# diffqc/dqc

Hardware: AMD Instinct MI355X
Metric: SCF iterations/sec (Fock build + XC grid) per GPU, cc-pVDZ 20-atom (higher is better)
Workload: dtype f64

## Files before the change

### dqc_amd/batch.py

```python
from typing import Callable, List, Sequence

import torch
import torch.distributed as dist


def molecule_cost(nao: int, ngrid: int) -> float:
    return float(nao) ** 4 + 12.0 * float(ngrid) * float(nao) ** 2


def molecule_bytes(nao: int, ngrid: int, ncomp: int = 4) -> int:
    nb = (nao + 7) // 8
    npair = nb * (nb + 1) // 2
    ld = (nao + 15) // 16 * 16 + 16
    return npair * (npair + 1) // 2 * 4096 * 8 + 8 * ncomp * ngrid * ld + 8 * 16 * ngrid + 64 * ld * ld


def reserve_device_memory(nbytes: int, device) -> float:
    import time
    dev = torch.device(device)
    free, _ = torch.cuda.mem_get_info(dev)
    cached = torch.cuda.memory_reserved(dev) - torch.cuda.memory_allocated(dev)
    nbytes = int(min(nbytes, free - (2 << 30)))
    if nbytes <= cached:
        return 0.0
    torch.cuda.synchronize(dev)
    t0 = time.perf_counter()
    block = torch.empty(nbytes, dtype=torch.uint8, device=dev)
    del block
    return time.perf_counter() - t0
# ... 170 lines not shown
```

### dqc_amd/csrc/common.hpp

```cpp
#pragma once
#include <hip/hip_runtime.h>
#include <cmath>
#include <cstdint>
#include <cstdio>
#include <cstring>
#include <mutex>
#include <string>
#include <vector>

#include "../../include/dqc_amd.h"

#define DQC_LMAX 4
#define DQC_TILE_B 8
#define DQC_TILE_SZ 4096

namespace dqc {

__host__ __device__ inline int tile_dim(bool diag) { return diag ? 36 : 64; }
__host__ __device__ inline int tile_pidx(bool diag, int a, int b) {
    if (!diag) return a * 8 + b;
    const int hi = a > b ? a : b, lo = a > b ? b : a;
    return hi * (hi + 1) / 2 + lo;
}
__host__ __device__ inline long long tile_row_off(long long I, long long J) {
// ... 129 lines not shown
        void *p = nullptr;
        if (dmalloc(&p, n * sizeof(T) + 8)) return DQC_ENOMEM;
        *dst = (T *)p;
        return 0;
    }
    void release() {
        for (void *p : ptrs) (void)(async ? hipFreeAsync(p, ast) : hipFree(p));
        ptrs.clear();
        for (Staging *s : stg) staging_release(s, ast);
        stg.clear();
    }
    ~DevPool() { release(); }
};

int upload_shells(DevShells &d, const Basis &b, DevPool &pool, hipStream_t st);

inline int ncart(int l) { return (l + 1) * (l + 2) / 2; }

struct SideStreams {
    static constexpr int MAX = 4;
    hipStream_t s[MAX] = {};
    hipEvent_t ev_fork = nullptr, ev_join[MAX] = {};
    int n = 0, next = 0;
    hipStream_t take() { return s[next++ % n]; }
    int fork(hipStream_t st) {
        if (hipEventRecord(ev_fork, st) != hipSuccess) return DQC_EHIP;
        for (int i = 0; i < n; i++)
            if (hipStreamWaitEvent(s[i], ev_fork, 0) != hipSuccess) return DQC_EHIP;
        return DQC_OK;
    }
// ... 172 lines not shown
```

### dqc_amd/csrc/grid_density.hip

```cpp
#include "grid_common.hpp"

namespace dqc {

constexpr int DEN_BM = 64;
constexpr int DEN_NT = DEN_BM * 4;
constexpr int DEN_KC = 16;
constexpr int DEN_SA = DEN_KC + 2;

#ifdef DEN_TRACE
__device__ long long g_den_trace[4 * 16384];
DQC_DEV void den_trace(int k) {
    if (threadIdx.x == 0 && blockIdx.x < 16384) {
        if (k == 0) {
            unsigned hw, xcc;
            asm volatile("s_getreg_b32 %0, hwreg(HW_REG_HW_ID)" : "=s"(hw));
            asm volatile("s_getreg_b32 %0, hwreg(HW_REG_XCC_ID)" : "=s"(xcc));
            g_den_trace[4 * blockIdx.x + 3] = (long long)(((xcc & 7u) << 8) | ((hw >> 8) & 0xffu));
        }
        g_den_trace[4 * blockIdx.x + k] = wall_clock64();
    }
}
#define DEN_TRACE_POINT(k) den_trace(k)
#else
#define DEN_TRACE_POINT(k)
// ... 571 lines not shown
    unsigned n = 0;
    while (__hip_atomic_load(flag, __ATOMIC_ACQUIRE, __HIP_MEMORY_SCOPE_WORKGROUP) < want) {
        if (__hip_atomic_load(broken, __ATOMIC_RELAXED, __HIP_MEMORY_SCOPE_WORKGROUP) != 0u) break;
        if (++n > ROLE_SPIN_CAP) {
            __hip_atomic_store(broken, 1u, __ATOMIC_RELAXED, __HIP_MEMORY_SCOPE_WORKGROUP);
            break;
        }
        __builtin_amdgcn_s_sleep(2);
    }
}

DQC_DEV void role_signal(unsigned *flag, unsigned v) {
    __hip_atomic_store(flag, v, __ATOMIC_RELEASE, __HIP_MEMORY_SCOPE_WORKGROUP);
}

template <int NRT, int NT>
__global__ __launch_bounds__(ROLE_NT, 1) void density_roles_kernel(double *__restrict__ rho, double *__restrict__ grho,
                                                                   const double *__restrict__ ao, int ngrid,
                                                                   const double *__restrict__ orbt, int lda) {
    using G = RoleGeom<NRT, NT>;
    constexpr int RP = G::RP, S = G::S, P0 = G::P0, P1 = G::P1, LD = NT * 16;
    constexpr int NPF = 4;
    static_assert(NT >= 2 && NT <= 14 && P1 >= 1, "one epilogue panel of 2..14 tiles");
    extern __shared__ __attribute__((aligned(16))) double lds[];
    double *sLT = lds, *sMB = lds + G::LT_SZ, *sAall = sMB + 4 * G::MB_W;
    unsigned *flags = reinterpret_cast<unsigned *>(sAall + 4 * G::SA_W);
    const int tid = threadIdx.x, lane = tid & 63;
    const int wave = __builtin_amdgcn_readfirstlane(tid >> 6);
    const int lr = lane & 15, lk = lane >> 4;
    const int ntiles = (ngrid + DEN_BM - 1) / DEN_BM;
    const size_t cs = (size_t)ngrid * lda;

    for (int e = tid; e < RP * LD; e += ROLE_NT) {
        const int r = e / LD, c = e - r * LD;
        sLT[r * S + c] = orbt[e];
    }
    if (tid < 16) flags[tid] = 0u;
    __syncthreads();
    const int w = wave & 3;
    unsigned *filled = flags + w, *drained = flags + 4 + w, *broken = flags + 8;
    double *mb = sMB + w * G::MB_W + lane * 2;
    unsigned seq = 0;

    if (wave < 4) {
        double *sA = sAall + w * G::SA_W;
        const int arow = lane >> 2, aseg = (lane & 3) * 4;
        double2 pa0a, pa0b, pa1a, pa1b, pa2a, pa2b, pa3a, pa3b;
        static_assert(NPF == 4, "four named prefetch sets");
#define DQC_ROLE_REQUEST(T, KC, SET)                                                                       \
    {                                                         \
        const int rmax_ = ngrid - 1 - (T) * DEN_BM;                                                        \
        const double *s_ = ao + (size_t)(T) * DEN_BM * lda + (min(w * 16 + arow, rmax_) * lda + aseg) + (KC) * DEN_KC; \
// ... 61 lines not shown
                    }
                role_wait(drained, seq, broken);
#pragma unroll
                for (int ct = 0; ct < PMAX; ct++)
                    if (ct < (h ? P1 : P0)) {
                        *reinterpret_cast<double2 *>(mb + (2 * ct) * 128) = make_double2(acc[ct][0], acc[ct][1]);
                        *reinterpret_cast<double2 *>(mb + (2 * ct + 1) * 128) = make_double2(acc[ct][2], acc[ct][3]);
                    }
                seq++;
                role_signal(filled, seq);
            }
        }
#undef DQC_ROLE_REQUEST4
#undef DQC_ROLE_STEP
#undef DQC_ROLE_REQUEST
    } else {
        for (int t = blockIdx.x; t < ntiles; t += gridDim.x) {
            const int g0 = t * DEN_BM;
            const int rmax = ngrid - 1 - g0;
            const double *aoblk = ao + (size_t)g0 * lda;
            int roff[4];
#pragma unroll
            for (int r = 0; r < 4; r++) roff[r] = min(w * 16 + lk + 4 * r, rmax) * lda + 2 * lr;
            v4d acc[NT];
#pragma unroll
            for (int h = 0; h < 2; h++) {
                role_wait(filled, seq + 1, broken);
#pragma unroll
                for (int ct = 0; ct < (h ? P1 : P0); ct++) {
                    const double2 lo = *reinterpret_cast<const double2 *>(mb + (2 * ct) * 128);
// ... 25 lines not shown
#pragma unroll
                for (int r = 0; r < 4; r++) {
                    const int row = g0 + w * 16 + lk + 4 * r;
                    if (row < ngrid) {
                        const double nan = __builtin_nan("");
                        grho[row] = bad ? nan : 2.0 * p[r][1];
                        grho[(size_t)ngrid + row] = bad ? nan : 2.0 * p[r][2];
                        grho[2 * (size_t)ngrid + row] = bad ? nan : 2.0 * p[r][3];
                    }
                }
            }
        }
    }
}

static bool density_roles_shape(int nrt, int ntile) { return nrt == 3 && ntile == 13; }

static bool density_roles_enabled() {
    const char *e = getenv("DQC_DENSITY_ROLES");
    return !(e && e[0] == '0');
}

static int launch_density_roles(int nrt, int ntile, hipStream_t st, double *rho, double *grho, const double *ao, int ngrid,
                                const double *orbt, int lda) {
    static int ncu = 0;
    if (ncu == 0) {
        int dev = 0, n = 0;
        if (hipGetDevice(&dev) != hipSuccess || hipDeviceGetAttribute(&n, hipDeviceAttributeMultiprocessorCount, dev) != hipSuccess || n <= 0) {
            set_error("density_roles: cannot read the device's CU count");
            return DQC_EINVAL;
        }
        ncu = n;
    }
    const int ntiles = (ngrid + DEN_BM - 1) / DEN_BM;
    if (nrt == 3 && ntile == 13) {
        constexpr size_t shm = RoleGeom<3, 13>::lds_bytes();
        static_assert(shm <= 160 * 1024, "one block has to fit the CU's LDS");
        auto kern = density_roles_kernel<3, 13>;
        (void)hipFuncSetAttribute((const void *)kern, hipFuncAttributeMaxDynamicSharedMemorySize, (int)shm);
        hipLaunchKernelGGL(kern, dim3(std::min(ntiles, ncu)), dim3(ROLE_NT), shm, st, rho, grho, ao, ngrid, orbt, lda);
        return 0;
    }
    set_error("density_roles: internal shape dispatch error");
    return DQC_EINVAL;
}

template <int NRT>
__global__ __launch_bounds__(256, 2) void density_lr_tau_kernel(double *__restrict__ rho, double *__restrict__ grho, double *__restrict__ tau,
                                                                const double *__restrict__ ao, int ngrid, int ld,
                                                                const double *__restrict__ orb, int lda) {
    extern __shared__ __attribute__((aligned(16))) double lds[];
    constexpr int RP = LrGeom<NRT>::RP, RPS = LrGeom<NRT>::RPS;
    constexpr int A_SZ = DEN_BM * DEN_SA, B_SZ = DEN_KC * RPS;
    constexpr int NL2 = (DEN_KC * RP / 2 + DEN_NT - 1) / DEN_NT;
    static_assert(NL2 <= 4, "L chunk wider than 4 double2 per thread");
    double *sA = lds, *sB = lds + 4 * A_SZ;
    const int tid = threadIdx.x, wave = tid >> 6, lane = tid & 63;
    const int lr = lane & 15, lk = lane >> 4;
    const int g0 = blockIdx.x * DEN_BM;
// ... 210 lines not shown
    const int lim = gga ? dqc::lr_max_nct(norb_pad / 16) : 16;
    const int nchunk = (ntile + lim - 1) / lim;
    const int nct = (ntile + nchunk - 1) / nchunk;
    dim3 grid((ngrid + DEN_BM - 1) / DEN_BM);
    int rc;
    if (gga && density_roles_shape(norb_pad / 16, ntile) && density_roles_enabled())
        rc = launch_density_roles(norb_pad / 16, ntile, st, d_rho, d_grho, d_ao, ngrid, d_orbt, lda);
    else
        rc = gga ? launch_density_lr<true>(norb_pad / 16, nct, grid, st, d_rho, d_grho, d_ao, ngrid, ld, d_orb, d_orbt, ntile, lda)
                 : launch_density_lr<false>(norb_pad / 16, nct, grid, st, d_rho, d_grho, d_ao, ngrid, ld, d_orb, d_orbt, ntile, lda);
    if (rc) return rc;
    DQC_CHECK_LAUNCH();
    return DQC_OK;
}

int dqc_grid_density_lr_roles(int nao, int norb_pad, int gga) {
    using namespace dqc;
    if (!gga || norb_pad <= 0 || dqc_padded_norb(norb_pad) != norb_pad) return 0;
    return density_roles_shape(norb_pad / 16, dqc_padded_nao(nao) / 16) && density_roles_enabled() ? 1 : 0;
}

int dqc_grid_density_lr_pol(double *d_rho, double *d_grho, const double *d_ao, int ncomp, int ngrid, int nao,
                            const double *d_orb, const double *d_orbt, int norb_pad_spin, void *stream) {
    using namespace dqc;
    hipStream_t st = (hipStream_t)stream;
    if (ngrid <= 0) return DQC_OK;
    if (!d_grho || ncomp < 4) { set_error("dqc_grid_density_lr_pol: needs the four AO components and the gradient output"); return DQC_EINVAL; }
    if (norb_pad_spin != 16 && norb_pad_spin != 32 && norb_pad_spin != 48 && norb_pad_spin != 64) {
        set_error("dqc_grid_density_lr_pol: norb_pad_spin must be 16, 32, 48 or 64");
        return DQC_EINVAL;
// ... 65 lines not shown
```

### dqc_amd/csrc/gto.hip

```cpp
#include "common.hpp"
#include <type_traits>

namespace dqc {

namespace gto_ce {
#define C2S_QUAL constexpr
#include "cart2sph.inc"
#undef C2S_QUAL
}

typedef double gto_v2d __attribute__((ext_vector_type(2)));
template <int DERIV>
__global__ __launch_bounds__(64) void eval_gto_kernel(double *__restrict__ out, const double *__restrict__ coords,
                                                       int ngrid, int nao, int ld, DevShells sh, int colrange) {
    constexpr int NC = DERIV == 0 ? 1 : (DERIV == 1 ? 4 : (DERIV == 2 ? 5 : 10));
    constexpr int GTO_CW = DERIV == 0 ? 16 : 8;
    __shared__ double tile[1][NC][64][GTO_CW + 1];
    constexpr int wave = 0;
    const int lane = threadIdx.x;
    const int g0 = blockIdx.x * 64;
    if (g0 >= ngrid) return;
    const int g = min(g0 + lane, ngrid - 1);
    const double px = coords[g * 3], py = coords[g * 3 + 1], pz = coords[g * 3 + 2];
    const size_t cstride = (size_t)ngrid * ld;

    const int cbeg = blockIdx.y * colrange, cend = min(cbeg + colrange, ld);
// ... 89 lines not shown
            if (nfill == GTO_CW) {
                flush(GTO_CW);
                col0 += GTO_CW;
                nfill = 0;
            }
        }
    };
    static_assert(DQC_LMAX == 4, "one shell body per accepted l");

    for (int is = 0; is < sh.nsh; is++) {
        const int l = sh.l[is], np = sh.nprim[is], po = sh.prim_off[is];
        const int a0 = sh.ao_off[is];
        if (a0 + 2 * l + 1 <= cbeg || a0 >= cend) continue;
        const double x = px - sh.xyz[is * 3], y = py - sh.xyz[is * 3 + 1], z = pz - sh.xyz[is * 3 + 2];
        const double r2 = x * x + y * y + z * z;
        double e0 = 0, e1 = 0, e2 = 0;
        for (int ip = 0; ip < np; ip++) {
            double a = sh.exps[po + ip];
            double e = sh.coefs[po + ip] * exp(-a * r2);
            e0 += e;
            e1 -= 2.0 * a * e;
            e2 += 4.0 * a * a * e;
        }
        switch (l) {
        case 0: shell(std::integral_constant<int, 0>{}, a0, x, y, z, e0, e1, e2); break;
        case 1: shell(std::integral_constant<int, 1>{}, a0, x, y, z, e0, e1, e2); break;
        case 2: shell(std::integral_constant<int, 2>{}, a0, x, y, z, e0, e1, e2); break;
        case 3: shell(std::integral_constant<int, 3>{}, a0, x, y, z, e0, e1, e2); break;
        default: shell(std::integral_constant<int, 4>{}, a0, x, y, z, e0, e1, e2); break;
        }
    }
    while (col0 + nfill < cend) {
        for (int c = 0; c < NC; c++) tile[wave][c][lane][nfill] = 0.0;
        nfill++;
        if (nfill == GTO_CW) {
            flush(GTO_CW);
            col0 += GTO_CW;
            nfill = 0;
// ... 25 lines not shown
        const int ncomp = deriv == 0 ? 1 : (deriv == 1 ? 4 : (deriv == 2 ? 5 : 10));
        const size_t body = (size_t)ncomp * (size_t)ngrid * ld, slack = dqc_ao_doubles(ncomp, ngrid, b.nao) - body;
        if (slack) DQC_HIP(hipMemsetAsync(d_out + body, 0, slack * sizeof(double), st));
        if (deriv == 0)
            hipLaunchKernelGGL(eval_gto_kernel<0>, grid, dim3(64), 0, st, d_out, d_coords, ngrid, b.nao, ld, ds, colrange);
        else if (deriv == 1)
            hipLaunchKernelGGL(eval_gto_kernel<1>, grid, dim3(64), 0, st, d_out, d_coords, ngrid, b.nao, ld, ds, colrange);
        else if (deriv == 2)
            hipLaunchKernelGGL(eval_gto_kernel<2>, grid, dim3(64), 0, st, d_out, d_coords, ngrid, b.nao, ld, ds, colrange);
        else
            hipLaunchKernelGGL(eval_gto_kernel<3>, grid, dim3(64), 0, st, d_out, d_coords, ngrid, b.nao, ld, ds, colrange);
        DQC_CHECK_LAUNCH();
    }
    return DQC_OK;
}
```

### dqc_amd/hamilton.py

```python
from collections import namedtuple
from typing import List, Optional

import os

import torch

from . import lib
from .basis import make_tables
from .linop import LinearOperator
from .utils.datastruct import AtomCGTOBasis, SpinParam, ValGrad
from .xc import LibXC

_COULOMB_SIDE = {}


def register_coulomb_side_stream(grid_stream, side_stream):
    key = (grid_stream.device.index, grid_stream.cuda_stream)
    if side_stream is None:
        _COULOMB_SIDE.pop(key, None)
    else:
        _COULOMB_SIDE[key] = side_stream


class _Memo:
# ... 238 lines not shown
                cached = (idx, int(idx.shape[0]))
                try:
                    grid._live_index_cache = cached
                except AttributeError:
                    pass
            if cached[1] < self.ngrid_full:
                self.live_index = cached[0]
                self.rgrid = self.rgrid[self.live_index].contiguous()
                self.dvolume = self.dvolume[self.live_index].contiguous()
        if self._pworld > 1:
            g = self.rgrid.shape[0]
            lo, hi = g * self._prank // self._pworld, g * (self._prank + 1) // self._pworld
            self.rgrid, self.dvolume = self.rgrid[lo:hi].contiguous(), self.dvolume[lo:hi].contiguous()
        deriv = {1: 0, 2: 1, 4: 2}[self.xcfamily]
        self._ao = lib.eval_gto(self._tab, self.rgrid, deriv)
        self.is_grid_set = True
        self.is_ao_set = True
        self.is_grad_ao_set = deriv >= 1
        self.is_lapl_ao_set = deriv == 2
        self._ao_lapl_pm = None

    def grid_select(self, x):
        return x if self.live_index is None else x[..., self.live_index]

    def grid_scatter(self, x):
        if self.live_index is None:
            return x
        out = torch.zeros(tuple(x.shape[:-1]) + (self.ngrid_full,), dtype=x.dtype, device=x.device)
        out[..., self.live_index] = x
        return out
# ... 342 lines not shown
        if not self.is_ao_set:
            raise RuntimeError("Please call `setup_grid(grid, xc)` first")
        gga = self.xcfamily in (2, 4)
        if gga and not self.is_grad_ao_set:
            raise RuntimeError("Please call `setup_grid(grid, gradlevel>=1)` to calculate the density gradient")
        fac = self._factor_of(dm)
        use_factor = fac is not None and (self.xcfamily != 4 or self.is_lapl_ao_set)
        self.grid_path_counts["factor" if use_factor else "dense"] += 1
        if use_factor and self.xcfamily == 4 and isinstance(self.xc, LibXC) and all(f[0].shape[1] <= 96 for f in fac):
            rho, grho, kin = lib.grid_density_lr_tau(self._ao, self._nao_ao, fac[0])
            for f in fac[1:]:
                r2, g2, k2 = lib.grid_density_lr_tau(self._ao, self._nao_ao, f)
                rho, grho, kin = rho + r2, grho + g2, kin + k2
            return ValGrad(value=rho, grad=grho, lapl=None, kin=kin)
        if use_factor:
            rho, grho = lib.grid_density_lr(self._ao, self._nao_ao, fac[0], gga)
            for f in fac[1:]:
                r2, g2 = lib.grid_density_lr(self._ao, self._nao_ao, f, gga)
                rho = rho + r2
                grho = None if grho is None else grho + g2
            if self.xcfamily != 4:
                return ValGrad(value=rho, grad=grho)
            gg = sum(lib.grid_density_lr(self._ao[d], self._nao_ao, f, False)[0] for d in (1, 2, 3) for f in fac)
            if isinstance(self.xc, LibXC):
                return ValGrad(value=rho, grad=grho, lapl=None, kin=gg * 0.5)
            if getattr(self, "_ao_lapl_pm", None) is None:
                self._ao_lapl_pm = (lib.ao_from(self._ao[0] + self._ao[4], self._nao_ao), lib.ao_from(self._ao[0] - self._ao[4], self._nao_ao))
            pl = sum(lib.grid_density_lr(self._ao_lapl_pm[0], self._nao_ao, f, False)[0] for f in fac)
            mi = sum(lib.grid_density_lr(self._ao_lapl_pm[1], self._nao_ao, f, False)[0] for f in fac)
            return ValGrad(value=rho, grad=grho, lapl=2.0 * (0.25 * (pl - mi) + gg), kin=gg * 0.5)
        dmdmt = (dm + dm.transpose(-2, -1)) * 0.5
        dao = lib.pad_matrix(self._unconvert_dm(dmdmt), self._ld)
        rho, grho = lib.grid_density(self._ao, self._nao_ao, dao, gga)
        if self.xcfamily != 4:
            return ValGrad(value=rho, grad=grho)
        if not self.is_lapl_ao_set:
            raise RuntimeError("Please call `setup_grid(grid, gradlevel>=2)` to calculate the density gradient")
        gg = sum(lib.grid_density_pair(self._ao[d], self._ao[d], self._nao_ao, dao) for d in (1, 2, 3))
        lb = lib.grid_density_pair(self._ao[0], self._ao[4], self._nao_ao, dao)
        return ValGrad(value=rho, grad=grho, lapl=(lb + gg) * 2, kin=gg * 0.5)

    def _dm2densinfo_pol(self, dm: SpinParam) -> SpinParam:
        if self.xcfamily == 2 and self.is_ao_set and self.is_grad_ao_set:
            fu, fd = self._factor_of(dm.u), self._factor_of(dm.d)
            if fu is not None and fd is not None and len(fu) == 1 and len(fd) == 1:
                out = lib.grid_density_lr_pol(self._ao, self._nao_ao, fu[0], fd[0])
                if out is not None:
                    self.grid_path_counts["factor"] += 2
                    self.grid_path_counts["factor_spin_fused"] = self.grid_path_counts.get("factor_spin_fused", 0) + 1
                    rho, grho = out
                    return SpinParam(u=ValGrad(value=rho[0], grad=grho[0]), d=ValGrad(value=rho[1], grad=grho[1]))
        return SpinParam(u=self._dm2densinfo(dm.u), d=self._dm2densinfo(dm.d))

    def _get_vxc_from_potinfo(self, potinfo: ValGrad):
        return self._sym_orth(self._vxc_ao_from_potinfo(potinfo)[:self._nao_ao, :self._nao_ao])

# ... 191 lines not shown
```

### dqc_amd/lib.py

```python
import ctypes
import os

import numpy as np
import torch

_HERE = os.path.dirname(os.path.abspath(__file__))
_LIBPATH = os.environ.get("DQC_AMD_LIB") or os.path.join(_HERE, "libdqc_amd.so")
_lib = None

XC_IDS = {"lda_x": 1, "lda_c_vwn": 7, "lda_c_pw": 12, "lda_c_pw_mod": 13, "gga_x_pbe": 101, "gga_x_pbe_r": 102, "gga_x_b88": 106,
          "gga_x_pbe_sol": 116, "gga_x_rpbe": 117, "gga_c_pbe": 130, "gga_c_lyp": 131, "gga_c_pbe_sol": 133,
          "mgga_x_scan": 263, "mgga_c_scan": 267, "mgga_x_tpss": 202, "mgga_c_tpss": 231,
          "lda_c_pz": 9, "gga_x_b86": 103, "gga_x_g96": 107, "gga_x_pw86": 108, "gga_x_pw91": 109, "gga_x_optx": 110, "gga_x_wc": 118,
          "gga_c_p86": 132}


class DqcAmdError(RuntimeError):
    pass


def libpath():
    return _LIBPATH


# ... 58 lines not shown
    lib.dqc_orth_factor_batched.argtypes = [c_dp, c_dp, c_dp, c_int, c_int, c_int, c_vp]
    lib.dqc_diis_solve.argtypes = [c_dp, c_dp, c_int, c_int, c_int, c_vp]
    lib.dqc_diis_solve_dev.argtypes = [c_dp, c_dp, c_int, c_int, c_vp, c_vp]
    lib.dqc_projector_work_doubles.argtypes = [c_int, c_int]
    lib.dqc_projector_work_doubles.restype = c_sz
    lib.dqc_projector_tc2.argtypes = [c_dp, c_dp, c_dp, c_int, ctypes.c_double, c_int, ctypes.c_double, c_dp, c_vp]
    lib.dqc_purify_tc2_persist.argtypes = [c_dp, c_dp, c_int, ctypes.c_double, c_int, ctypes.c_double, c_dp, c_vp, c_vp]
    lib.dqc_df_coulomb.argtypes = [c_dp, c_dp, c_dp, c_dp, c_int, c_int, c_dp, c_vp]
    lib.dqc_eri_tiles_to_dense.argtypes = [c_dp, c_dp, c_int, c_vp]
    lib.dqc_jk_from_tiles.argtypes = [c_dp, c_dp, c_dp, c_dp, c_int, c_dp, c_vp]
    lib.dqc_jk_multi_work_doubles.argtypes = [c_int, c_int, c_int]
    lib.dqc_jk_multi_work_doubles.restype = c_sz
    lib.dqc_jk_from_tiles_multi.argtypes = [c_dp, c_dp, c_int, c_dp, c_dp, c_int, c_dp, c_int, c_dp, c_vp]
    lib.dqc_eval_gto.argtypes = [c_int, c_dp, c_dp, c_int] + tab + [c_vp]
    lib.dqc_grid_density.argtypes = [c_dp, c_dp, c_dp, c_int, c_int, c_int, c_dp, c_vp]
    lib.dqc_xc_eval.argtypes = [c_dp, c_dp, c_dp, c_dp, c_dp, c_int, ip, dp, c_int, c_vp]
    lib.dqc_xc_eval_quad.argtypes = [c_dp, c_dp, c_dp, c_dp, c_dp, c_dp, c_dp, c_int, ip, dp, c_int, c_vp]
    lib.dqc_xc_eval_pol.argtypes = [c_dp] * 9 + [c_int, ip, dp, c_int, c_vp]
    lib.dqc_xc_eval_mgga.argtypes = [c_dp] * 7 + [c_int, ip, dp, c_int, c_vp]
    lib.dqc_xc_eval_mgga_pol.argtypes = [c_dp] * 11 + [c_int, ip, dp, c_int, c_vp]
    lib.dqc_xc_eval_mgga_pol2.argtypes = [c_dp] * 12 + [c_int, ip, dp, c_int, c_vp]
    lib.dqc_stream_create_partition.argtypes = [ctypes.POINTER(c_vp), c_int, c_int, c_int]
    lib.dqc_stream_destroy.argtypes = [c_vp]
    lib.dqc_stream_cus.argtypes = [c_vp]
    lib.dqc_set_vxc_cus.argtypes = [c_int]
    lib.dqc_fock_factor.argtypes = [c_dp, c_dp, c_dp, c_dp, c_int, c_dp, c_int, c_int, c_int, c_int, c_int, c_vp]
    lib.dqc_fock_orb2dm.argtypes = [c_dp, c_dp, c_dp, c_dp, c_dp, c_int, c_dp, c_int, c_int, c_int, c_int, c_int, c_vp]
    lib.dqc_grid_vxc_raw.argtypes = [c_dp, c_dp, c_int, c_int, c_int, c_dp, c_dp, c_dp, dp, c_vp]
    lib.dqc_fock_finish_vraw.argtypes = [c_dp, c_dp, c_dp, c_dp, c_int, ctypes.c_double, c_dp, c_dp, c_int, c_int, c_vp]
    lib.dqc_fock_prep.argtypes = [c_dp, c_dp, c_dp, c_dp, c_int, c_int, c_int, c_int, c_vp]
# ... 540 lines not shown

def eval_gto(tab, rgrid, deriv):
    ngrid = rgrid.shape[0]
    ncomp = {0: 0, 1: 4, 2: 5, 3: 10}[deriv]
    nc = max(ncomp, 1)
    lda = ao_stride(tab.nao)
    flat = torch.empty(int(load().dqc_ao_doubles(nc, int(ngrid), int(tab.nao))), dtype=torch.float64, device=rgrid.device)
    out = flat[:nc * ngrid * lda].view(nc, ngrid, lda)
    out = out[0] if ncomp == 0 else out
    with _on(rgrid.device) as st_:
        _check(load().dqc_eval_gto(deriv, _ptr(out), _ptr(rgrid.contiguous()), ngrid, *tab.args(), st_),
               "dqc_eval_gto")
    return out


def pad_matrix(m, ld):
    n = m.shape[-1]
    if n == ld:
        return m.contiguous()
    out = torch.zeros((ld, ld), dtype=m.dtype, device=m.device)
    out[:n, :n] = m
    return out


def grid_density(ao, nao, dm_pad, gga):
    ncomp = 1 if ao.dim() == 2 else ao.shape[0]
    ngrid = ao.shape[-2]
    rho = torch.empty(ngrid, dtype=torch.float64, device=ao.device)
    grho = torch.empty((3, ngrid), dtype=torch.float64, device=ao.device) if gga else None
    with _on(ao.device) as st_:
# ... 277 lines not shown
```

### include/dqc_amd.h

```cpp
#ifndef DQC_AMD_H
#define DQC_AMD_H
#include <stddef.h>
#include <stdint.h>

#ifdef __cplusplus
extern "C" {
#endif

#define DQC_OK 0
#define DQC_EINVAL (-1)
#define DQC_EHIP (-2)
#define DQC_ENOMEM (-3)

const char *dqc_last_error(void);
int dqc_version(void);
int dqc_nao(const int *bas, int nbas);
int dqc_padded_nao(int nao);
int dqc_ao_stride(int nao);
size_t dqc_ao_doubles(int ncomp, int ngrid, int nao);

int dqc_int1e(int which, double *d_out, const int *atm, int natm, const int *bas, int nbas,
              const double *env, int nenv, const double *zs, void *stream);

size_t dqc_eri_tile_count(int nao);
// ... 118 lines not shown
int dqc_orth_factor(double *d_q, const double *d_y, const double *d_g, int n, int r, void *stream);

int dqc_purify_tc2_batched(double *d_x, double *d_tmp, int ld, int nmol, double nocc, int iters, double tol,
                           double *d_state, void *stream);
int dqc_orth_factor_batched(double *d_q, const double *d_y, const double *d_g, int n, int r, int nmol, void *stream);
int dqc_diis_solve(double *d_c, const double *d_gram, int nmol, int nhist, int m, void *stream);
int dqc_diis_solve_dev(double *d_c, const double *d_gram, int nmol, int nhist, const long long *d_count, void *stream);

int dqc_grid_vxc(double *d_vmat, const double *d_ao, int ncomp, int ngrid, int nao,
                 const double *d_w, const double *d_vrho, const double *d_vgrad, void *stream);

int dqc_padded_norb(int norb);
int dqc_grid_density_lr(double *d_rho, double *d_grho, const double *d_ao, int ncomp, int ngrid, int nao,
                        const double *d_orb, const double *d_orbt, int norb_pad, void *stream);
int dqc_grid_density_lr_roles(int nao, int norb_pad, int gga);
int dqc_grid_density_lr_pol(double *d_rho, double *d_grho, const double *d_ao, int ncomp, int ngrid, int nao,
                            const double *d_orb, const double *d_orbt, int norb_pad_spin, void *stream);

int dqc_grid_xc_gradient_terms(double *d_q, double *d_perao, const double *d_ao, int ngrid, int nao, const double *d_b,
                               const double *d_c0, const double *d_c1, const double *d_c2, int ldb, const double *d_w,
                               const double *d_vrho, const double *d_u, const double *d_grho, const double *d_vtau, void *stream);

int dqc_grid_density_lr_tau(double *d_rho, double *d_grho, double *d_tau, const double *d_ao, int ncomp, int ngrid, int nao,
                            const double *d_orb, int norb_pad, void *stream);

int dqc_grid_density_pair(double *d_out, const double *d_ao_a, const double *d_ao_b, int ngrid, int nao,
                          const double *d_dm, void *stream);
int dqc_grid_vxc_pair(double *d_vmat, const double *d_ao_a, const double *d_ao_b, int ngrid, int nao,
                      const double *d_w, const double *d_v, void *stream);

// ... 40 lines not shown
```

Baseline: 796.4.

## Compute density gradient from cached radial GTO terms instead of AO gradient tables

Adds a radial table (per grid point and shell slot, the contracted exponential and its derivative) evaluated once at grid setup. A new variant of the roles density kernel rebuilds the angular derivative parts on the fly from point coordinates and compile-time cart-to-spherical coefficients, then dots them with the orbital-factor products. This avoids streaming the three AO gradient components from memory on each SCF iteration. The cost is extra arithmetic per point and extra LDS for the table, and the path only applies to one padded shape (13 tiles, l<=2, GGA).

```diff
diff --git a/dqc_amd/batch.py b/dqc_amd/batch.py
--- a/dqc_amd/batch.py
+++ b/dqc_amd/batch.py
@@ -11,8 +11,12 @@
 def molecule_bytes(nao: int, ngrid: int, ncomp: int = 4) -> int:
     nb = (nao + 7) // 8
     npair = nb * (nb + 1) // 2
-    ld = (nao + 15) // 16 * 16 + 16
-    return npair * (npair + 1) // 2 * 4096 * 8 + 8 * ncomp * ngrid * ld + 8 * 16 * ngrid + 64 * ld * ld
+    ld = (nao + 15) // 16 * 16
+    lda = (nao + 7) // 8 * 8
+    rows = 36 * nb + 64 * (npair - nb)
+    tiles = rows * (rows + 64) // 2 * 8
+    radial = 16 * ngrid * min(160, (nao // 2 + 8 + 15) // 16 * 16) if ncomp == 4 and ld // 16 == 13 else 0
+    return tiles + 8 * ncomp * ngrid * lda + 8 * 16 * ngrid + 64 * (ld + 16) * (ld + 16) + radial
 
 
 def reserve_device_memory(nbytes: int, device) -> float:
diff --git a/dqc_amd/csrc/common.hpp b/dqc_amd/csrc/common.hpp
--- a/dqc_amd/csrc/common.hpp
+++ b/dqc_amd/csrc/common.hpp
@@ -167,6 +167,9 @@
 };
 
 int upload_shells(DevShells &d, const Basis &b, DevPool &pool, hipStream_t st);
+
+constexpr int RADIAL_HDR = 8, RADIAL_REC = 6, RADIAL_MAX_SLOTS = 160;
+int build_radial_table(const Basis &b, std::vector<double> &table);
 
 inline int ncart(int l) { return (l + 1) * (l + 2) / 2; }
 
diff --git a/dqc_amd/csrc/grid_density.hip b/dqc_amd/csrc/grid_density.hip
--- a/dqc_amd/csrc/grid_density.hip
+++ b/dqc_amd/csrc/grid_density.hip
@@ -609,10 +609,132 @@
     __hip_atomic_store(flag, v, __ATOMIC_RELEASE, __HIP_MEMORY_SCOPE_WORKGROUP);
 }
 
-template <int NRT, int NT>
-__global__ __launch_bounds__(ROLE_NT, 1) void density_roles_kernel(double *__restrict__ rho, double *__restrict__ grho,
-                                                                   const double *__restrict__ ao, int ngrid,
-                                                                   const double *__restrict__ orbt, int lda) {
+namespace den_ce {
+#define C2S_QUAL constexpr
+#include "cart2sph.inc"
+#undef C2S_QUAL
+}
+
+template <int l>
+DQC_DEV void radial_shell_terms(const double *rec, const double *mbp, double px, double py, double pz, double e0, double e1,
+                                double &gx, double &gy, double &gz) {
+    const double x = px - rec[0], y = py - rec[1], z = pz - rec[2];
+    const int *off = reinterpret_cast<const int *>(rec + 3);
+    double xp[l + 2], yp[l + 2], zp[l + 2];
+    xp[0] = yp[0] = zp[0] = 1.0;
+#pragma unroll
+    for (int k = 1; k <= l + 1; k++) { xp[k] = xp[k - 1] * x; yp[k] = yp[k - 1] * y; zp[k] = zp[k - 1] * z; }
+    constexpr int nc = (l + 1) * (l + 2) / 2, ns = 2 * l + 1;
+#pragma unroll
+    for (int m = 0; m < ns; m++) {
+        const int o = off[m];
+        const double bq = mbp[o < 0 ? 0 : o];
+        const double b = o < 0 ? 0.0 : bq;
+        double vx = 0, vy = 0, vz = 0;
+        int c = 0;
+#pragma unroll
+        for (int lx = l; lx >= 0; lx--)
+#pragma unroll
+            for (int ly = l - lx; ly >= 0; ly--, c++) {
+                const double cf = den_ce::C2S[den_ce::C2S_OFF[l] + m * nc + c];
+                if (cf == 0.0) continue;
+                const int lz = l - lx - ly;
+                vx += cf * ((lx ? lx * xp[lx ? lx - 1 : 0] : 0.0) * yp[ly] * zp[lz] * e0 + xp[lx + 1] * yp[ly] * zp[lz] * e1);
+                vy += cf * ((ly ? ly * yp[ly ? ly - 1 : 0] : 0.0) * xp[lx] * zp[lz] * e0 + xp[lx] * yp[ly + 1] * zp[lz] * e1);
+                vz += cf * ((lz ? lz * zp[lz ? lz - 1 : 0] : 0.0) * xp[lx] * yp[ly] * e0 + xp[lx] * yp[ly] * zp[lz + 1] * e1);
+            }
+        gx += b * vx;
+        gy += b * vy;
+        gz += b * vz;
+    }
+}
+
+DQC_DEV void role_radial_rowdots(double *__restrict__ grho, const double *__restrict__ rad, const double *__restrict__ coords,
+                                 int ngrid, int nslot, const double *sTB, const double *mbw, int w, int lane, unsigned *filled,
+                                 unsigned *drained, unsigned *broken) {
+    const int pt = lane >> 2, k = lane & 3;
+    const int ntiles = (ngrid + DEN_BM - 1) / DEN_BM;
+    const int *hdr = reinterpret_cast<const int *>(sTB);
+    const int nstep0 = __builtin_amdgcn_readfirstlane(hdr[1]);
+    const int se0 = __builtin_amdgcn_readfirstlane(hdr[2]), pe0 = __builtin_amdgcn_readfirstlane(hdr[3]);
+    const int se1 = __builtin_amdgcn_readfirstlane(hdr[4]), pe1 = __builtin_amdgcn_readfirstlane(hdr[5]);
+    const int nch = nslot >> 4;
+    const double *mbp = mbw + (pt >> 3) * 128 + (pt & 3) * 32 + ((pt >> 2) & 1);
+    const double *recs = sTB + RADIAL_HDR + k * RADIAL_REC;
+    const double2 *rad2 = reinterpret_cast<const double2 *>(rad);
+
+    int t = blockIdx.x, c = 0;
+    int tp = blockIdx.x, cp = 0;
+    unsigned seq = 0;
+    double px = 0, py = 0, pz = 0, gx = 0, gy = 0, gz = 0;
+    double2 s0[4], s1[4], s2[4];
+#pragma unroll
+    for (int i = 0; i < 4; i++) s0[i] = s1[i] = s2[i] = make_double2(0.0, 0.0);
+
+    auto request = [&](double2(&s)[4]) {
+        if (tp < ntiles) {
+            const int row = tp * DEN_BM + min(w * 16 + pt, ngrid - 1 - tp * DEN_BM);
+            const double2 *src = rad2 + (size_t)row * nslot + cp * 16 + k;
+#pragma unroll
+            for (int i = 0; i < 4; i++) s[i] = src[i * 4];
+        }
+        if (++cp == nch) { cp = 0; tp += gridDim.x; }
+    };
+    auto work = [&](const double2(&s)[4]) {
+        if (c == 0) {
+            const int row = t * DEN_BM + min(w * 16 + pt, ngrid - 1 - t * DEN_BM);
+            px = coords[(size_t)row * 3], py = coords[(size_t)row * 3 + 1], pz = coords[(size_t)row * 3 + 2];
+            gx = gy = gz = 0.0;
+            role_wait(filled, seq + 1, broken);
+        }
+#pragma unroll
+        for (int i = 0; i < 4; i++) {
+            const int step = c * 4 + i;
+            if (step == nstep0) {
+                seq++;
+                role_signal(drained, seq);
+                role_wait(filled, seq + 1, broken);
+            }
+            const int cls = step < nstep0 ? (step < se0 ? 0 : (step < pe0 ? 1 : 2)) : (step < se1 ? 0 : (step < pe1 ? 1 : 2));
+            const double *rec = recs + step * (4 * RADIAL_REC);
+            switch (cls) {
+            case 0: radial_shell_terms<0>(rec, mbp, px, py, pz, s[i].x, s[i].y, gx, gy, gz); break;
+            case 1: radial_shell_terms<1>(rec, mbp, px, py, pz, s[i].x, s[i].y, gx, gy, gz); break;
+            default: radial_shell_terms<2>(rec, mbp, px, py, pz, s[i].x, s[i].y, gx, gy, gz); break;
+            }
+        }
+        if (++c == nch) {
+            seq++;
+            role_signal(drained, seq);
+            gx += __shfl_xor(gx, 1); gy += __shfl_xor(gy, 1); gz += __shfl_xor(gz, 1);
+            gx += __shfl_xor(gx, 2); gy += __shfl_xor(gy, 2); gz += __shfl_xor(gz, 2);
+            const bool bad = __hip_atomic_load(broken, __ATOMIC_RELAXED, __HIP_MEMORY_SCOPE_WORKGROUP) != 0u;
+            const int row = t * DEN_BM + w * 16 + pt;
+            if (k == 0 && row < ngrid) {
+                const double nan = __builtin_nan("");
+                grho[row] = bad ? nan : 2.0 * gx;
+                grho[(size_t)ngrid + row] = bad ? nan : 2.0 * gy;
+                grho[2 * (size_t)ngrid + row] = bad ? nan : 2.0 * gz;
+            }
+            c = 0;
+            t += gridDim.x;
+        }
+    };
+    request(s0);
+    request(s1);
+    while (t < ntiles) {
+        request(s2); work(s0);
+        if (t >= ntiles) break;
+        request(s0); work(s1);
+        if (t >= ntiles) break;
+        request(s1); work(s2);
+    }
+}
+
+template <int NRT, int NT, bool RADIAL>
+DQC_DEV void density_roles_body(double *__restrict__ rho, double *__restrict__ grho, const double *__restrict__ ao, int ngrid,
+                                const double *__restrict__ orbt, int lda, const double *__restrict__ rad,
+                                const double *__restrict__ coords, const double *__restrict__ rtab, int nslot) {
     using G = RoleGeom<NRT, NT>;
     constexpr int RP = G::RP, S = G::S, P0 = G::P0, P1 = G::P1, LD = NT * 16;
     constexpr int NPF = 4;
@@ -631,6 +753,9 @@
         sLT[r * S + c] = orbt[e];
     }
     if (tid < 16) flags[tid] = 0u;
+    double *sTB = reinterpret_cast<double *>(flags + 16);
+    if constexpr (RADIAL)
+        for (int e = tid; e < RADIAL_HDR + nslot * RADIAL_REC; e += ROLE_NT) sTB[e] = rtab[e];
     __syncthreads();
     const int w = wave & 3;
     unsigned *filled = flags + w, *drained = flags + 4 + w, *broken = flags + 8;
@@ -722,6 +847,8 @@
 #undef DQC_ROLE_REQUEST4
 #undef DQC_ROLE_STEP
 #undef DQC_ROLE_REQUEST
+    } else if constexpr (RADIAL) {
+        role_radial_rowdots(grho, rad, coords, ngrid, nslot, sTB, sMB + w * G::MB_W, w, lane, filled, drained, broken);
     } else {
         for (int t = blockIdx.x; t < ntiles; t += gridDim.x) {
             const int g0 = t * DEN_BM;
@@ -777,6 +904,23 @@
     }
 }
 
+template <int NRT, int NT>
+__global__ __launch_bounds__(ROLE_NT, 1) void density_roles_kernel(double *__restrict__ rho, double *__restrict__ grho,
+                                                                   const double *__restrict__ ao, int ngrid,
+                                                                   const double *__restrict__ orbt, int lda) {
+    density_roles_body<NRT, NT, false>(rho, grho, ao, ngrid, orbt, lda, nullptr, nullptr, nullptr, 0);
+}
+
+template <int NRT, int NT>
+__global__ __launch_bounds__(ROLE_NT, 1) void density_roles_radial_kernel(double *__restrict__ rho, double *__restrict__ grho,
+                                                                          const double *__restrict__ ao, int ngrid,
+                                                                          const double *__restrict__ orbt, int lda,
+                                                                          const double *__restrict__ rad,
+                                                                          const double *__restrict__ coords,
+                                                                          const double *__restrict__ rtab, int nslot) {
+    density_roles_body<NRT, NT, true>(rho, grho, ao, ngrid, orbt, lda, rad, coords, rtab, nslot);
+}
+
 static bool density_roles_shape(int nrt, int ntile) { return nrt == 3 && ntile == 13; }
 
 static bool density_roles_enabled() {
@@ -806,6 +950,83 @@
     }
     set_error("density_roles: internal shape dispatch error");
     return DQC_EINVAL;
+}
+
+static bool density_radial_enabled() {
+    const char *e = getenv("DQC_DENSITY_RADIAL");
+    return !(e && e[0] == '0');
+}
+
+static int launch_density_roles_radial(hipStream_t st, double *rho, double *grho, const double *ao, int ngrid, const double *orbt,
+                                       int lda, const double *rad, const double *coords, const double *rtab, int nslot) {
+    static int ncu = 0;
+    if (ncu == 0) {
+        int dev = 0, n = 0;
+        if (hipGetDevice(&dev) != hipSuccess || hipDeviceGetAttribute(&n, hipDeviceAttributeMultiprocessorCount, dev) != hipSuccess || n <= 0) {
+            set_error("density_roles_radial: cannot read the device's CU count");
+            return DQC_EINVAL;
+        }
+        ncu = n;
+    }
+    const int ntiles = (ngrid + DEN_BM - 1) / DEN_BM;
+    constexpr size_t shm_max = RoleGeom<3, 13>::lds_bytes() + sizeof(double) * (RADIAL_HDR + RADIAL_MAX_SLOTS * RADIAL_REC);
+    static_assert(shm_max <= 160 * 1024, "one block with the largest radial table has to fit the CU's LDS");
+    const size_t shm = RoleGeom<3, 13>::lds_bytes() + sizeof(double) * (RADIAL_HDR + (size_t)nslot * RADIAL_REC);
+    auto kern = density_roles_radial_kernel<3, 13>;
+    (void)hipFuncSetAttribute((const void *)kern, hipFuncAttributeMaxDynamicSharedMemorySize, (int)shm_max);
+    hipLaunchKernelGGL(kern, dim3(std::min(ntiles, ncu)), dim3(ROLE_NT), shm, st, rho, grho, ao, ngrid, orbt, lda, rad, coords,
+                       rtab, nslot);
+    return 0;
+}
+
+int build_radial_table(const Basis &b, std::vector<double> &table) {
+    constexpr int NT = 13, P0 = RoleGeom<3, NT>::P0;
+    table.clear();
+    if (dqc_padded_nao(b.nao) / 16 != NT || b.grouped()) return 0;
+    for (const HostShell &h : b.shells)
+        if (h.l > 2) return 0;
+    struct Slot { int shell; int off[5]; };
+    std::vector<Slot> slots;
+    int bound[2][3];
+    for (int h = 0; h < 2; h++)
+        for (int l = 0; l <= 2; l++) {
+            for (int is = 0; is < (int)b.shells.size(); is++) {
+                const HostShell &s = b.shells[is];
+                if (s.l != l) continue;
+                Slot sl{is, {-1, -1, -1, -1, -1}};
+                bool any = false;
+                for (int m = 0; m < 2 * l + 1; m++) {
+                    const int col = s.ao_off + m;
+                    const int ct = col < 32 * (NT / 2) ? 2 * (col >> 5) + (col & 1) : col >> 4;
+                    const int lr = col < 32 * (NT / 2) ? (col & 31) >> 1 : col & 15;
+                    if ((ct < P0) != (h == 0)) continue;
+                    sl.off[m] = (ct - h * P0) * 256 + 2 * lr;
+                    any = true;
+                }
+                if (any) slots.push_back(sl);
+            }
+            const bool last = h == 1 && l == 2;
+            while (slots.size() % (last ? 16 : 4)) slots.push_back(Slot{-1, {-1, -1, -1, -1, -1}});
+            bound[h][l] = (int)slots.size() / 4;
+        }
+    const int nslot = (int)slots.size();
+    if (nslot > RADIAL_MAX_SLOTS) return 0;
+    table.assign(RADIAL_HDR + (size_t)nslot * RADIAL_REC, 0.0);
+    int *hdr = reinterpret_cast<int *>(table.data());
+    hdr[0] = nslot;
+    hdr[1] = bound[0][2];
+    hdr[2] = bound[0][0]; hdr[3] = bound[0][1];
+    hdr[4] = bound[1][0]; hdr[5] = bound[1][1];
+    for (int i = 0; i < nslot; i++) {
+        double *rec = table.data() + RADIAL_HDR + (size_t)i * RADIAL_REC;
+        const Slot &sl = slots[i];
+        if (sl.shell >= 0)
+            for (int d = 0; d < 3; d++) rec[d] = b.shells[sl.shell].r[d];
+        int *ri = reinterpret_cast<int *>(rec + 3);
+        for (int m = 0; m < 5; m++) ri[m] = sl.off[m];
+        ri[5] = sl.shell;
+    }
+    return nslot;
 }
 
 template <int NRT>
@@ -1046,6 +1267,26 @@
     return DQC_OK;
 }
 
+int dqc_grid_density_lr_radial(double *d_rho, double *d_grho, const double *d_ao, int ngrid, int nao, const double *d_radial,
+                               const double *d_table, int nslot, const double *d_coords, const double *d_orbt, int norb_pad,
+                               void *stream) {
+    using namespace dqc;
+    hipStream_t st = (hipStream_t)stream;
+    if (ngrid <= 0) return DQC_OK;
+    if (norb_pad <= 0 || dqc_padded_norb(norb_pad) != norb_pad) {
+        set_error("dqc_grid_density_lr_radial: norb_pad must be a value returned by dqc_padded_norb");
+        return DQC_EINVAL;
+    }
+    const int ntile = dqc_padded_nao(nao) / 16;
+    if (!d_grho || !d_radial || !d_table || !d_coords || nslot < 16 || nslot % 16 || nslot > RADIAL_MAX_SLOTS ||
+        !density_roles_shape(norb_pad / 16, ntile) || !density_radial_enabled())
+        return 1;
+    int rc = launch_density_roles_radial(st, d_rho, d_grho, d_ao, ngrid, d_orbt, dqc_ao_stride(nao), d_radial, d_coords, d_table, nslot);
+    if (rc) return rc;
+    DQC_CHECK_LAUNCH();
+    return DQC_OK;
+}
+
 int dqc_grid_density_lr_roles(int nao, int norb_pad, int gga) {
     using namespace dqc;
     if (!gga || norb_pad <= 0 || dqc_padded_norb(norb_pad) != norb_pad) return 0;
diff --git a/dqc_amd/csrc/gto.hip b/dqc_amd/csrc/gto.hip
--- a/dqc_amd/csrc/gto.hip
+++ b/dqc_amd/csrc/gto.hip
@@ -10,6 +10,33 @@
 }
 
 typedef double gto_v2d __attribute__((ext_vector_type(2)));
+
+DQC_DEV void gto_radial(const DevShells &sh, int po, int np, double r2, double &e0, double &e1, double &e2) {
+    e0 = 0, e1 = 0, e2 = 0;
+    for (int ip = 0; ip < np; ip++) {
+        double a = sh.exps[po + ip];
+        double e = sh.coefs[po + ip] * exp(-a * r2);
+        e0 += e;
+        e1 -= 2.0 * a * e;
+        e2 += 4.0 * a * a * e;
+    }
+}
+
+__global__ __launch_bounds__(256) void gto_radial_kernel(double *__restrict__ out, const double *__restrict__ coords, int ngrid,
+                                                         int nslot, const double *__restrict__ table, DevShells sh) {
+    const size_t idx = (size_t)blockIdx.x * 256 + threadIdx.x;
+    if (idx >= (size_t)ngrid * nslot) return;
+    const int g = (int)(idx / nslot), slot = (int)(idx - (size_t)g * nslot);
+    const int is = reinterpret_cast<const int *>(table + RADIAL_HDR + (size_t)slot * RADIAL_REC + 3)[5];
+    double e0 = 0, e1 = 0, e2 = 0;
+    if (is >= 0) {
+        const double px = coords[g * 3], py = coords[g * 3 + 1], pz = coords[g * 3 + 2];
+        const double x = px - sh.xyz[is * 3], y = py - sh.xyz[is * 3 + 1], z = pz - sh.xyz[is * 3 + 2];
+        const double r2 = x * x + y * y + z * z;
+        gto_radial(sh, sh.prim_off[is], sh.nprim[is], r2, e0, e1, e2);
+    }
+    __builtin_nontemporal_store(gto_v2d{e0, e1}, reinterpret_cast<gto_v2d *>(out) + idx);
+}
 template <int DERIV>
 __global__ __launch_bounds__(64) void eval_gto_kernel(double *__restrict__ out, const double *__restrict__ coords,
                                                        int ngrid, int nao, int ld, DevShells sh, int colrange) {
@@ -129,14 +156,8 @@
         if (a0 + 2 * l + 1 <= cbeg || a0 >= cend) continue;
         const double x = px - sh.xyz[is * 3], y = py - sh.xyz[is * 3 + 1], z = pz - sh.xyz[is * 3 + 2];
         const double r2 = x * x + y * y + z * z;
-        double e0 = 0, e1 = 0, e2 = 0;
-        for (int ip = 0; ip < np; ip++) {
-            double a = sh.exps[po + ip];
-            double e = sh.coefs[po + ip] * exp(-a * r2);
-            e0 += e;
-            e1 -= 2.0 * a * e;
-            e2 += 4.0 * a * a * e;
-        }
+        double e0, e1, e2;
+        gto_radial(sh, po, np, r2, e0, e1, e2);
         switch (l) {
         case 0: shell(std::integral_constant<int, 0>{}, a0, x, y, z, e0, e1, e2); break;
         case 1: shell(std::integral_constant<int, 1>{}, a0, x, y, z, e0, e1, e2); break;
@@ -192,3 +213,39 @@
     }
     return DQC_OK;
 }
+
+extern "C" int dqc_radial_layout(const int *atm, int natm, const int *bas, int nbas, const double *env, int nenv, int *info) {
+    using namespace dqc;
+    Basis b;
+    int rc = parse_basis(b, atm, natm, bas, nbas, env, nenv, nullptr);
+    if (rc) return rc;
+    std::vector<double> table;
+    const int nslot = build_radial_table(b, table);
+    info[0] = nslot > 0 ? 1 : 0;
+    info[1] = nslot;
+    info[2] = (int)table.size();
+    return DQC_OK;
+}
+
+extern "C" int dqc_eval_gto_radial(double *d_out, double *d_table, const double *d_coords, int ngrid, const int *atm,
+                                   int natm, const int *bas, int nbas, const double *env, int nenv, void *stream) {
+    using namespace dqc;
+    hipStream_t st = (hipStream_t)stream;
+    Basis b;
+    int rc = parse_basis(b, atm, natm, bas, nbas, env, nenv, nullptr);
+    if (rc) return rc;
+    std::vector<double> table;
+    const int nslot = build_radial_table(b, table);
+    if (nslot <= 0) { set_error("dqc_eval_gto_radial: the basis has no radial table (dqc_radial_layout: not served)"); return DQC_EINVAL; }
+    DevPool pool(st);
+    DevShells ds;
+    if ((rc = upload_shells(ds, b, pool, st))) { set_error("dqc_eval_gto_radial: device upload failed"); return rc; }
+    if ((rc = pool.copy_to(d_table, table, st))) { set_error("dqc_eval_gto_radial: table upload failed"); return rc; }
+    if (ngrid > 0) {
+        const size_t n = (size_t)ngrid * nslot;
+        hipLaunchKernelGGL(gto_radial_kernel, dim3((unsigned)((n + 255) / 256)), dim3(256), 0, st, d_out, d_coords, ngrid, nslot,
+                           d_table, ds);
+        DQC_CHECK_LAUNCH();
+    }
+    return DQC_OK;
+}
diff --git a/dqc_amd/hamilton.py b/dqc_amd/hamilton.py
--- a/dqc_amd/hamilton.py
+++ b/dqc_amd/hamilton.py
@@ -276,6 +276,7 @@
             self.rgrid, self.dvolume = self.rgrid[lo:hi].contiguous(), self.dvolume[lo:hi].contiguous()
         deriv = {1: 0, 2: 1, 4: 2}[self.xcfamily]
         self._ao = lib.eval_gto(self._tab, self.rgrid, deriv)
+        self._radial = lib.eval_gto_radial(self._tab, self.rgrid) if deriv == 1 and self.rgrid.shape[0] > 0 else None
         self.is_grid_set = True
         self.is_ao_set = True
         self.is_grad_ao_set = deriv >= 1
@@ -648,9 +649,9 @@
                 rho, grho, kin = rho + r2, grho + g2, kin + k2
             return ValGrad(value=rho, grad=grho, lapl=None, kin=kin)
         if use_factor:
-            rho, grho = lib.grid_density_lr(self._ao, self._nao_ao, fac[0], gga)
+            rho, grho = self._density_lr(fac[0], gga)
             for f in fac[1:]:
-                r2, g2 = lib.grid_density_lr(self._ao, self._nao_ao, f, gga)
+                r2, g2 = self._density_lr(f, gga)
                 rho = rho + r2
                 grho = None if grho is None else grho + g2
             if self.xcfamily != 4:
@@ -674,6 +675,13 @@
         lb = lib.grid_density_pair(self._ao[0], self._ao[4], self._nao_ao, dao)
         return ValGrad(value=rho, grad=grho, lapl=(lb + gg) * 2, kin=gg * 0.5)
 
+    def _density_lr(self, f, gga):
+        if gga and getattr(self, "_radial", None) is not None:
+            out = lib.grid_density_lr_radial(self._ao, self._nao_ao, f, self._radial, self.rgrid)
+            if out is not None:
+                return out
+        return lib.grid_density_lr(self._ao, self._nao_ao, f, gga)
+
     def _dm2densinfo_pol(self, dm: SpinParam) -> SpinParam:
         if self.xcfamily == 2 and self.is_ao_set and self.is_grad_ao_set:
             fu, fd = self._factor_of(dm.u), self._factor_of(dm.d)
diff --git a/dqc_amd/lib.py b/dqc_amd/lib.py
--- a/dqc_amd/lib.py
+++ b/dqc_amd/lib.py
@@ -96,6 +96,9 @@
     lib.dqc_jk_from_tiles_multi.argtypes = [c_dp, c_dp, c_int, c_dp, c_dp, c_int, c_dp, c_int, c_dp, c_vp]
     lib.dqc_eval_gto.argtypes = [c_int, c_dp, c_dp, c_int] + tab + [c_vp]
     lib.dqc_grid_density.argtypes = [c_dp, c_dp, c_dp, c_int, c_int, c_int, c_dp, c_vp]
+    lib.dqc_radial_layout.argtypes = tab + [ip]
+    lib.dqc_eval_gto_radial.argtypes = [c_dp, c_dp, c_dp, c_int] + tab + [c_vp]
+    lib.dqc_grid_density_lr_radial.argtypes = [c_dp, c_dp, c_dp, c_int, c_int, c_dp, c_dp, c_int, c_dp, c_dp, c_int, c_vp]
     lib.dqc_xc_eval.argtypes = [c_dp, c_dp, c_dp, c_dp, c_dp, c_int, ip, dp, c_int, c_vp]
     lib.dqc_xc_eval_quad.argtypes = [c_dp, c_dp, c_dp, c_dp, c_dp, c_dp, c_dp, c_int, ip, dp, c_int, c_vp]
     lib.dqc_xc_eval_pol.argtypes = [c_dp] * 9 + [c_int, ip, dp, c_int, c_vp]
@@ -666,6 +669,40 @@
     return out
 
 
+def radial_layout(tab):
+    info = (ctypes.c_int * 3)()
+    _check(load().dqc_radial_layout(*tab.args(), info), "dqc_radial_layout")
+    return bool(info[0]), int(info[1]), int(info[2])
+
+
+def eval_gto_radial(tab, rgrid):
+    served, nslot, ntab = radial_layout(tab)
+    if not served:
+        return None
+    ngrid = rgrid.shape[0]
+    radial = torch.empty((ngrid, nslot, 2), dtype=torch.float64, device=rgrid.device)
+    table = torch.empty(ntab, dtype=torch.float64, device=rgrid.device)
+    with _on(rgrid.device) as st_:
+        _check(load().dqc_eval_gto_radial(_ptr(radial), _ptr(table), _ptr(rgrid.contiguous()), ngrid, *tab.args(), st_),
+               "dqc_eval_gto_radial")
+    return radial, table, nslot
+
+
+def grid_density_lr_radial(ao, nao, factor, radial, rgrid):
+    orb, orbt = factor
+    rad, table, nslot = radial
+    ngrid = ao.shape[-2]
+    rho = torch.empty(ngrid, dtype=torch.float64, device=ao.device)
+    grho = torch.empty((3, ngrid), dtype=torch.float64, device=ao.device)
+    with _on(ao.device) as st_:
+        rc = load().dqc_grid_density_lr_radial(_ptr(rho), _ptr(grho), _ptr(ao), ngrid, nao, _ptr(rad), _ptr(table), nslot,
+                                               _ptr(rgrid), _ptr(orbt), orb.shape[1], st_)
+        if rc == 1:
+            return None
+        _check(rc, "dqc_grid_density_lr")
+    return rho, grho
+
+
 def pad_matrix(m, ld):
     n = m.shape[-1]
     if n == ld:
diff --git a/include/dqc_amd.h b/include/dqc_amd.h
--- a/include/dqc_amd.h
+++ b/include/dqc_amd.h
@@ -156,6 +156,12 @@
 int dqc_grid_density_lr(double *d_rho, double *d_grho, const double *d_ao, int ncomp, int ngrid, int nao,
                         const double *d_orb, const double *d_orbt, int norb_pad, void *stream);
 int dqc_grid_density_lr_roles(int nao, int norb_pad, int gga);
+int dqc_radial_layout(const int *atm, int natm, const int *bas, int nbas, const double *env, int nenv, int *info);
+int dqc_eval_gto_radial(double *d_out, double *d_table, const double *d_coords, int ngrid, const int *atm,
+                        int natm, const int *bas, int nbas, const double *env, int nenv, void *stream);
+int dqc_grid_density_lr_radial(double *d_rho, double *d_grho, const double *d_ao, int ngrid, int nao, const double *d_radial,
+                               const double *d_table, int nslot, const double *d_coords, const double *d_orbt, int norb_pad,
+                               void *stream);
 int dqc_grid_density_lr_pol(double *d_rho, double *d_grho, const double *d_ao, int ncomp, int ngrid, int nao,
                             const double *d_orb, const double *d_orbt, int norb_pad_spin, void *stream);
 
```

Result: slower. 759.1 (-4.7%).
